# ebiggers/libdeflate

Measured on AMD Instinct MI355X. Metric: compress+decompress MB/s, 64 KiB chunks level 6, higher is better.
Workload: dtype u8

## Files before the change

### include/libdeflate_amd.h

```cpp
#ifndef LIBDEFLATE_AMD_H
#define LIBDEFLATE_AMD_H

#include <stddef.h>
#include <stdint.h>

#ifdef __cplusplus
extern "C" {
#endif

#define LIBDEFLATE_VERSION_MAJOR	1
#define LIBDEFLATE_VERSION_MINOR	25
#define LIBDEFLATE_VERSION_STRING	"1.25"
#define LIBDEFLATE_AMD_VERSION_STRING	"0.1-gfx950"

#ifndef LIBDEFLATEAPI
#  define LIBDEFLATEAPI __attribute__((visibility("default")))
#endif

struct libdeflate_compressor;
struct libdeflate_decompressor;

struct libdeflate_options {
	size_t sizeof_options;
	void *(*malloc_func)(size_t);
// ... 141 lines not shown
			      uint64_t *d_out_nbytes, void *stream);

LIBDEFLATEAPI int
libdeflate_amd_compress_batch_bounded(struct libdeflate_compressor *compressor,
				      int format, size_t n_chunks,
				      const void *d_in, const uint64_t *d_in_offsets,
				      const uint64_t *d_in_nbytes,
				      void *d_out, const uint64_t *d_out_offsets,
				      const uint64_t *d_out_avail,
				      uint64_t *d_out_nbytes, size_t max_in_nbytes,
				      void *stream);

LIBDEFLATEAPI void
libdeflate_amd_compress_last_schedule(const struct libdeflate_compressor *compressor,
				      uint32_t out[4]);

LIBDEFLATEAPI int
libdeflate_amd_decompress_batch(struct libdeflate_decompressor *decompressor,
				int format, size_t n_chunks,
				const void *d_in, const uint64_t *d_in_offsets,
				const uint64_t *d_in_nbytes,
				void *d_out, const uint64_t *d_out_offsets,
				const uint64_t *d_out_avail,
				int32_t *d_results,
				uint64_t *d_actual_in, uint64_t *d_actual_out,
				void *stream);

#define LIBDEFLATE_AMD_DICT_WINDOW 20480

LIBDEFLATEAPI int
// ... 439 lines not shown
```

### libdeflate_amd/api.py

```python
import collections
import ctypes
from ctypes import c_size_t, c_void_p

import numpy as np

from . import binding
from .binding import FORMATS, PREFIX, check


def _buf(b):
    if isinstance(b, np.ndarray):
        assert b.dtype == np.uint8 and b.flags["C_CONTIGUOUS"]
        return b.ctypes.data_as(c_void_p), b.size
    if isinstance(b, (bytes, bytearray, memoryview)):
        arr = np.frombuffer(b, dtype=np.uint8)
        return arr.ctypes.data_as(c_void_p), arr.size
    raise TypeError(type(b))


TarGz = collections.namedtuple("TarGz", "result nbytes seek_index windows words rows results")


class Compressor:

# ... 227 lines not shown
                self._h, FORMATS[fmt], in_offsets.numel(), data.data_ptr(),
                in_offsets.data_ptr(), in_nbytes.data_ptr(), out.data_ptr(),
                out_offsets.data_ptr(), out_avail.data_ptr(),
                out_nbytes.data_ptr(), _stream_ptr(stream)), "compress_batch")
        else:
            check(self._lib.libdeflate_amd_compress_batch_bounded(
                self._h, FORMATS[fmt], in_offsets.numel(), data.data_ptr(),
                in_offsets.data_ptr(), in_nbytes.data_ptr(), out.data_ptr(),
                out_offsets.data_ptr(), out_avail.data_ptr(),
                out_nbytes.data_ptr(), int(max_chunk), _stream_ptr(stream)),
                "compress_batch_bounded")

    def last_schedule(self):
        return binding.compress_last_schedule(self._h)

    def compress_dict(self, fmt, dictionary, data, out_avail=None):
        p, n = _buf(data)
        dp, dn = _buf(dictionary)
        if out_avail is None:
            out_avail = self.bound(fmt, n) + 4
        out = np.empty(max(out_avail, 1), dtype=np.uint8)
        r = self._lib.libdeflate_amd_compress_dict(
            self._h, FORMATS[fmt], dp, dn, p, n, out.ctypes.data_as(c_void_p), out_avail)
        if r == 0:
            return None
        return out[:r].tobytes()

    def compress_batch_dict(self, fmt, dictionary, data, in_offsets, in_nbytes, out,
                            out_offsets, out_avail, out_nbytes, stream=None):
        check(self._lib.libdeflate_amd_compress_batch_dict(
# ... 599 lines not shown
```

### libdeflate_amd/binding.py

```python
import ctypes
import os
from ctypes import (POINTER, c_char_p, c_int, c_int32, c_size_t, c_uint32,
                    c_uint64, c_void_p)

_HERE = os.path.dirname(os.path.abspath(__file__))
LIB_PATH = os.environ.get("LIBDEFLATE_AMD_LIB",
                          os.path.join(_HERE, "libdeflate_amd.so"))

SUCCESS, BAD_DATA, SHORT_OUTPUT, INSUFFICIENT_SPACE = 0, 1, 2, 3
FMT_DEFLATE, FMT_ZLIB, FMT_GZIP, FMT_BGZF = 0, 1, 2, 3
FORMATS = {"deflate": FMT_DEFLATE, "zlib": FMT_ZLIB, "gzip": FMT_GZIP, "bgzf": FMT_BGZF}
BGZF_BLOCK, BGZF_MEMBER_MAX, BGZF_EOF_BYTES, BGZF_NO_EOF = 65280, 65536, 28, 1
BGZF_MORE_MEMBERS, BGZF_HAS_EOF, BGZF_RESULT_WORDS, BGZF_VOFFSETS = 16, 1, 5, 2
GZM_MORE_MEMBERS, GZM_MORE_CANDIDATES, GZM_RESULT_WORDS, GZM_SLACK = 16, 17, 5, 1024
GZM_NAME_MAX = 65536
ZIP_MORE_ENTRIES, ZIP_MORE_CANDIDATES, ZIP_UNSUPPORTED = 16, 17, 18
ZIP_RESULT_WORDS, ZIP_WORDS, ZIP_SLACK, ZIP_ZIP64 = 5, 8, 1024, 1
ZIP_PIECE = 1 << 20
TAR_MORE_RECORDS, TAR_MORE_CANDIDATES, TAR_UNSUPPORTED = 16, 17, 18
TAR_RESULT_WORDS, TAR_WORDS, TAR_SLACK = 5, 8, 1024
TAR_EOF, TAR_HAS_L, TAR_HAS_PAX = 1, 2, 4
PNG_UNSUPPORTED, PNG_WORDS, PNG_LE16 = 18, 8, 1
PNG_FILTER_ADAPTIVE, PNGW_RESULT_WORDS = 5, 4
ZIP_STORE, ZIP_FORCE_ZIP64, ZIPW_RESULT_WORDS = 1, 2, 4
# ... 9 lines not shown
    "libdeflate_gzip_compress", "libdeflate_gzip_compress_bound",
    "libdeflate_free_compressor",
    "libdeflate_alloc_decompressor", "libdeflate_alloc_decompressor_ex",
    "libdeflate_deflate_decompress", "libdeflate_deflate_decompress_ex",
    "libdeflate_zlib_decompress", "libdeflate_zlib_decompress_ex",
    "libdeflate_gzip_decompress", "libdeflate_gzip_decompress_ex",
    "libdeflate_free_decompressor",
    "libdeflate_adler32", "libdeflate_crc32",
    "libdeflate_set_memory_allocator",
]
BATCH_SYMBOLS = [
    "libdeflate_amd_device_ready", "libdeflate_amd_last_error",
    "libdeflate_amd_reload_env",
    "libdeflate_amd_compress_batch", "libdeflate_amd_decompress_batch",
    "libdeflate_amd_compress_batch_bounded", "libdeflate_amd_compress_last_schedule",
    "libdeflate_amd_crc32_batch", "libdeflate_amd_adler32_batch",
    "libdeflate_amd_compress_batch_host",
    "libdeflate_amd_decompress_batch_host",
    "libdeflate_amd_compact_offsets_len", "libdeflate_amd_compact_batch",
    "libdeflate_amd_gzip_decompress_members",
    "libdeflate_amd_stream_stats", "libdeflate_amd_last_fanout",
    "libdeflate_amd_selfcheck",
    "libdeflate_amd_compress_batch_dict", "libdeflate_amd_decompress_batch_dict",
    "libdeflate_amd_compress_dict", "libdeflate_amd_decompress_dict_ex",
    "libdeflate_amd_bgzf_compress_bound", "libdeflate_amd_bgzf_compress_batch",
    "libdeflate_amd_bgzf_compress",
    "libdeflate_amd_bgzf_decompress_batch", "libdeflate_amd_bgzf_index_batch",
    "libdeflate_amd_bgzf_read_batch", "libdeflate_amd_bgzf_decompress",
    "libdeflate_amd_decompress_sizes_batch", "libdeflate_amd_decompress_sizes_batch_dict",
    "libdeflate_amd_decompress_sizes_batch_host", "libdeflate_amd_decompress_batch_packed",
# ... 58 lines not shown
        sig(f"libdeflate_{f}_decompress", c_int, P, P, SZ, P, SZ, psz)
        sig(f"libdeflate_{f}_decompress_ex", c_int, P, P, SZ, P, SZ, psz, psz)
    sig("libdeflate_crc32", c_uint32, c_uint32, P, SZ)
    sig("libdeflate_adler32", c_uint32, c_uint32, P, SZ)
    sig("libdeflate_set_memory_allocator", None, P, P)
    sig("libdeflate_amd_device_ready", c_int)
    sig("libdeflate_amd_last_error", c_char_p)
    sig("libdeflate_amd_reload_env", None)
    sig("libdeflate_amd_crc32_batch", c_int, SZ, P, P, P, P, P, P)
    sig("libdeflate_amd_adler32_batch", c_int, SZ, P, P, P, P, P, P)
    sig("libdeflate_amd_compress_batch", c_int, P, c_int, SZ, P, P, P, P, P,
        P, P, P)
    sig("libdeflate_amd_compress_batch_bounded", c_int, P, c_int, SZ, P, P, P, P, P,
        P, P, SZ, P)
    sig("libdeflate_amd_compress_last_schedule", None, P, POINTER(c_uint32))
    sig("libdeflate_amd_decompress_batch", c_int, P, c_int, SZ, P, P, P, P, P,
        P, P, P, P, P)
    sig("libdeflate_amd_compress_batch_host", c_int, P, c_int, SZ, P, P, P, P,
        P)
    sig("libdeflate_amd_decompress_batch_host", c_int, P, c_int, SZ, P, P, P,
        P, P, P, P)
    sig("libdeflate_amd_gzip_decompress_members", c_int, P, P, SZ, P, SZ, psz, psz, psz)
    sig("libdeflate_amd_stream_stats", None, POINTER(c_uint64))
    sig("libdeflate_amd_last_fanout", c_size_t)
    sig("libdeflate_amd_selfcheck", c_int, POINTER(c_uint64))
    sig("libdeflate_amd_compact_offsets_len", SZ, SZ)
    sig("libdeflate_amd_compact_batch", c_int, SZ, P, P, P, P, P, P)
    sig("libdeflate_amd_compress_batch_dict", c_int, P, c_int, SZ, P, SZ, P, P, P, P,
        P, P, P, P)
    sig("libdeflate_amd_decompress_batch_dict", c_int, P, c_int, SZ, P, SZ, P, P, P, P,
# ... 77 lines not shown
    out = (c_uint64 * 16)()
    load().libdeflate_amd_stream_stats(out)
    keys = ("parallel", "why_not", "filter_a", "blocks_found", "chunks_planned",
            "repairs", "chunks_decoded", "bytes", "us_in", "us_find", "us_count",
            "us_decode", "us_sum", "us_out", "windows", "host_chunks")
    return dict(zip(keys, [int(v) for v in out]))


def compress_last_schedule(compressor):
    out = (c_uint32 * 4)()
    load().libdeflate_amd_compress_last_schedule(compressor, out)
    return {"split": int(out[0]), "overlapped": int(out[1]), "head": int(out[2]),
            "tail": int(out[3])}


def last_error():
    return load().libdeflate_amd_last_error().decode()


def check(rc, what):
    if rc != 0:
        raise RuntimeError(f"{what} failed (status {rc}): {last_error()}")
```

### libdeflate_amd/csrc/deflate_kernel.hip

```cpp
#include <stddef.h>
#include "device_common.h"
#include "kernels.h"


#ifndef NT
#define NT LDA_DEFLATE_THREADS
#endif
#define VPT (1024 / NT)
#define NWAVES (NT / 64)
#ifndef TILE
#define TILE 4096
#endif
#ifndef RING
#define RING 32768u
#endif
#define RMASK (RING - 1)
#define LOOKAHEAD 272u
#ifndef HASH_BITS
#define HASH_BITS 13
#endif
#ifndef HASH3_BITS
#define HASH3_BITS 12
#endif
#define MAX_BLOCK_LEN 65536u
// ... 1414 lines not shown
	const u64 delta = ((u64)row16_sum(df >> 16) << 16) + row16_sum(df & 0xFFFF);
	bool sp = nprev && walkpos - block_start >= 5000 &&
		  delta >= (u64)nnew * 200 / 512 * nprev;
	if (fit_split && walkpos - block_start >= 5000)
		sp = true;
	wave_sync();
	if (lane < 10)
		L->obs[0][lane] = sp ? 0 : now;
	if (lane == 0)
		L->vars[V_SPLIT] = !sp ? 0 :
			L->vars[V_WPOS_PRE] - block_start >= 5000 ? 2 : 1;
}



static __device__ __forceinline__ u64 claim_buffer(lds_t *L, u32 *next_chunk, u32 tid)
{
	__syncthreads();
	if (tid == 0)
		L->vars[V_TMP0] = atomicAdd(next_chunk, 1u);
	__syncthreads();
	return bcast_first(L->vars[V_TMP0]);
}

static __device__ __forceinline__ void buffer_lds_init(lds_t *L, u32 tid)
{
	for (u32 i = tid; i < (1u << HASH_BITS) / 2; i += NT)
		((u32 *)L->head)[i] = 0x80008000u;
	for (u32 i = tid; i < (1u << HASH3_BITS) / 2; i += NT)
		((u32 *)L->head3)[i] = 0x80008000u;
	for (u32 i = tid; i < 320; i += NT)
		L->freq[i] = 0;
	if (tid < 10)
		L->obs[0][tid] = 0;
	if (tid < TILE / 64 + 1)
		L->rdy[tid] = 0;
	for (u32 i = tid; i < STG_WORDS + 8; i += NT)
		stg_of(L)[i] = 0;
	if (tid < 8)
		L->M[tid] = 0;
	if (tid == 0) {
		L->vars[V_NSEQ] = 0;
		L->vars[V_ENTRY] = 0;
		L->vars[V_PFLAG] = 0;
	}
// ... 103 lines not shown
{
	insert_tile3(L, c3ins, tnend,
		     tnend + TILE < n ? tnend + TILE : n, n, lane);
	__builtin_amdgcn_fence(__ATOMIC_RELEASE, "workgroup");
}

static __device__ __forceinline__ void
px_minlen_ahead(lds_t *L, u32 tnend, u32 n, u32 dict_len, u32 loaded, u32 depth, bool use3, u32 lane)
{
	const u32 nd = wave_distinct_bytes(L, tnend,
		loaded - tnend < TILE ? loaded - tnend : TILE, lane);
	if (lane == 0)
		L->vars[V_MINLEN] = min_len_policy(nd, n - dict_len, depth, use3);
}

static __device__ __forceinline__ void
px_round_b_tail(lds_t *L, u32 t, u32 n, u32 lo_nxt, u32 ml_cur, u32 depth, u32 nice,
		u32 mode, s32 limit, u32 tail_n, u32 tail_e, u32 tail_gen, u32 lane, u32 wave)
{
	__builtin_amdgcn_s_setprio(2);
	if (64 * (wave - 1) < tail_n) {
		u32 nx;
		(void)rb_batch(L, t, n, lo_nxt, ml_cur, rb_trim_depth(depth), nice,
			       tail_e, tail_e != 0, tail_gen, lane, &nx);
	}
	__builtin_amdgcn_fence(__ATOMIC_RELEASE, "workgroup");
	if (lane == 0)
		atomicAdd((u32 *)&L->vars[V_TAILDONE], 1u);
	wait_lds_eq(L, V_TAILDONE, RB_TAIL_WAVES);
	stage_steps_cur_claimed(L, limit, mode, nice, lane);
// ... 76 lines not shown
	const u8 *__restrict__ in_base, const u64 *__restrict__ in_offsets,    \
	const u64 *__restrict__ in_nbytes, u8 *__restrict__ out_base,          \
	const u64 *__restrict__ out_offsets,                                   \
	const u64 *__restrict__ out_avail_arr, u64 *__restrict__ out_nbytes,   \
	const u32 *__restrict__ sums, u64 *__restrict__ seq_scratch,           \
	const u32 *__restrict__ seg_info, u32 *__restrict__ next_chunk,       \
	const u8 *__restrict__ dict_pre
#define DEFLATE_KERNEL_ARGS                                                    \
	lds_raw, n_chunks, format, level, depth, nice, mode, in_base,          \
	in_offsets, in_nbytes, out_base, out_offsets, out_avail_arr,           \
	out_nbytes, sums, seq_scratch, seg_info, next_chunk, dict_pre

template <bool OPT, bool SPLIT = false> static __device__ __forceinline__ void
deflate_batch_body(u8 *lds_raw, DEFLATE_KERNEL_PARAMS,
		   u32 *__restrict__ tok_buf = NULL, u32 *__restrict__ blk_buf = NULL,
		   u32 tok_stride = 0, u32 blk_stride = 0, u32 *__restrict__ fused_cnt = NULL)
{
	static_assert(!(OPT && SPLIT), "levels 10-12 keep the fused block end");
	lds_t *L = (lds_t *)(uintptr_t)0;
	const u32 tid = threadIdx.x;
	if ((u32)(uintptr_t)(__attribute__((address_space(3))) u8 *)lds_raw != 0)
		__builtin_trap();
	u64 *__restrict__ seqg = seq_scratch + (size_t)blockIdx.x * SEQ_STRIDE;
	u32 *__restrict__ msave = (u32 *)(seqg + SEQ_GCAP);
	u32 *__restrict__ fsave = msave + TILE + 8;
	u32 *__restrict__ bsave = fsave + 640;
	u16 *__restrict__ c3g = (u16 *)(bsave + 512);
	u32 tog = 0;
	PROF_DECL;

	for (u32 i = tid; i < 256; i += NT) {
		u32 sl, xb, xv;
		length_code(i + 3, &sl, &xb, &xv);
		L->lslot[i] = (u8)sl;
	}
	const u32 *__restrict__ only = !SPLIT && blk_buf ? blk_buf + LDA_BLK_LIST(n_chunks) : NULL;
	const u64 n_todo = only ? bcast_first(*fused_cnt) : n_chunks;
	for (;;) {
		const u64 i_todo = claim_buffer(L, next_chunk, tid);
		if (i_todo >= n_todo)
			break;
		const u64 c = only ? bcast_first(only[i_todo]) : i_todo;
		const u8 *inp = in_base + in_offsets[c];
		u64 n64 = in_nbytes[c];
		u32 *__restrict__ const tokg = SPLIT ? tok_buf + c * tok_stride : (u32 *)seqg;
		u32 *__restrict__ const blk_desc = SPLIT ?
			blk_buf + LDA_BLK_HDR_WORDS(n_chunks) + c * blk_stride * LDA_BLK_WORDS : NULL;
		u32 nblocks = 0, blk_tok0 = 0;
		const u32 sinfo = dict_pre ? (n64 ? ((const u32 *)dict_pre)[0] : 0x80000000u) :
				  seg_info ? seg_info[c] : 0x80000000u;
		const u32 dict_len = sinfo & 0xFFFFu;
		const u32 lo_min = (sinfo >> 16) & 0x7FFFu;
		const bool seg_last = sinfo >> 31;
		const u32 pre_len = dict_pre ? dict_len : 0;
// ... 13 lines not shown
				overflow = true;
		}

		if (os.avail <= hdr_bytes + ftr_bytes && (hdr_bytes + ftr_bytes))
			overflow = true;
		if (n64 > 0xFFFFFF00u)
			overflow = true;
#ifdef LDA_SMALL
		if (n64 > RING)
			overflow = true;
#endif
		const bool over_bound = SPLIT && n64 > tok_stride;
		if (over_bound)
			overflow = true;
		const u32 n = (u32)n64;

		__syncthreads();
		PROF_START();
		buffer_lds_init(L, tid);
		os.sg = (u64)(0 - ((uintptr_t)os.out & 15));
		os.bits = 0;
		__syncthreads();

		if (!SPLIT) {
			if (!overflow && hdr_bytes)
				put_container_header(L, &os, format, level, dict_pre, hdr_bytes, tid);
			__syncthreads();
			stg_save(L, &os);
		}

		u32 loaded = 0;
		u32 block_start = dict_len;
		u32 walkpos = dict_len;
		const bool aligned_in = ((uintptr_t)inp & 15) == 0;

		const bool stored_only = level == 0 ||
			n - dict_len <= (u32)(55 - 4 * (level > 12 ? 12 : level));
		u32 num_tiles = (n + TILE - 1) / TILE;
		if (num_tiles == 0)
			num_tiles = 1;
		if (pre_len && !stored_only && !overflow) {
			stage_prefix(L, dict_pre + 64, pre_len, tid);
			loaded = pre_len;
		}

		const bool ra_all = depth <= 4;
		const bool optm = OPT && mode == 3;
		const u32 rounds = optm || ra_all ? 0 : S3_ROUNDS;
		const u32 dlim3 = mode ? 8192u : 4096u;
		const u32 ra_depth = ra_all ? depth : S3_RA_DEPTH;
		const u32 ra_class = ra_all ? DC_FULL :
				     ra_depth >= (depth >> S3_HALF_SHIFT) ? DC_HALF : DC_SHALLOW;
// ... 29 lines not shown
			} else {
				AS3 u32 *const MX = (AS3 u32 *)L->nxtB;
				const struct tile_window w = tile_window_of(t, tend, tn, lo_min, last_tile);
				u16 *c3nxt = c3g + (it & 1) * (TILE + 8);
				u16 *c3ins = c3g + ((it + 1) & 1) * (TILE + 8);

				const bool wl_copies = cur_real && !optm && rounds && mx_pending;
				if (cur_real) {
					cur_results_to_m(L, MX, fsave, mx_pending, wl_copies, carryv, walkpos, tid);
					mx_pending = false;
					ml_cur = ml_nxt;
					PROF_MARK(6);
				}
				const u32 s0_want0 = (it + 2) * TILE + LOOKAHEAD;
				const u32 s0_want = s0_want0 < n ? s0_want0 : n;
				const u32 s0_p = (loaded & ~15u) + tid * 16;
				const bool s0_pre = aligned_in && s0_p < s0_want;
				uint4 s0_v = make_uint4(0, 0, 0, 0);
				if (s0_pre)
					s0_v = *(const uint4 *)(inp + s0_p);
				tail_n = 0;
				if (cur_real && !optm) {
					if (rounds) {
						const u32 wc = build_worklist(L, (AS3 u32 *)L->nxtB,
									      wl_copies ? (const AS3 u32 *)MX : NULL,
									      mode, nice, wq_limit, tid);
						PROF_MARK(39);
						if (wc) {
							AS3 u32 *tl = (AS3 u32 *)L->nxtB;
							search_queue(L, t, n, w.lo_cur, ml_cur, depth, nice,
								     (AS3 u32 *)L->nxtB, (AS3 u32 *)L->nxtA, wc, tid,
								     nxt_real, &tail_n, &tail_gen, &tl);
							if (tail_n && wave >= 1 && wave <= RB_TAIL_WAVES) {
								const u32 k = 64 * (wave - 1) + lane;
								tail_e = k < tail_n ? tl[k] : 0;
// ... 65 lines not shown
							L->M[i] = msave[i];
						if (tid == 0) {
							L->vars[V_ENTRY] = ent0;
							L->vars[V_NSEQ] = nseq0;
						}
						__syncthreads();
						opt_stage++;
					}
				}

				const struct s0_state s0 = stage_s0(L, MX, inp, aligned_in, s0_pre, s0_p, s0_v,
					s0_want, loaded, ml_nxt, cur_real, nxt_real, tail_n, it, tid);
				loaded = s0.loaded;
				ml_nxt = s0.ml_nxt;
				PROF_MARK(1);
				if (it == 0) {
					if (wave == NWAVES - 1)
						insert_tile(L, 0, tnend, n, lane);
					if (wave == NWAVES - 2 && use3) {
						insert_tile3(L, c3nxt, 0, tnend, n, lane);
						__builtin_amdgcn_fence(__ATOMIC_RELEASE, "workgroup");
					}
					if (wave == NWAVES - 3 && nxt_real) {
						const u32 nd = wave_distinct_bytes(L, 0, loaded < TILE ? loaded : TILE, lane);
						if (lane == 0)
							L->vars[V_MINLEN] = min_len_policy(nd, n - dict_len, depth, use3);
					}
					__syncthreads();
					if (nxt_real)
						ml_nxt = bcast_first(L->vars[V_MINLEN]);
					PROF_MARK(2);
				}
				__builtin_amdgcn_fence(__ATOMIC_ACQUIRE, "workgroup");

				{
					const bool do_p2 = cur_real && !optm;
					AS3 u32 *const Mo = cur_real ? MX : (AS3 u32 *)L->M;
					PROF_WDECL;
					PROF_W0();
					if (wave == NWAVES - 1) {
						px_insert_chains(L, have_ins, tnend, n, lane);
						PROF_W(24);
					} else if (wave == NWAVES - 2) {
						__builtin_amdgcn_s_setprio(2);
						if (have_ins && use3)
							px_insert3(L, c3ins, tnend, n, lane);
						__builtin_amdgcn_s_setprio(0);
						if (have_ins && tnend >= dict_len)
							px_minlen_ahead(L, tnend, n, dict_len, loaded, depth, use3, lane);
						PROF_W(25);
					} else if (wave == 0 && do_p2) {
						if (tail_n)
							wait_lds_eq(L, V_ST2DONE, TILE / 64);
						__builtin_amdgcn_s_setprio(3);
						parse_and_base(L, tokg, t, w.limit, mode, nice, lane);
						__builtin_amdgcn_fence(__ATOMIC_RELEASE, "workgroup");
						if (lane == 0)
							*(volatile AS3 u32 *)&L->vars[V_PFLAG] = it;
						__builtin_amdgcn_s_setprio(0);
						if (tail_n && nxt_real && lane < 4)
							Mo[lane] = L->M[TILE + lane];
						PROF_W(26);
					} else if (RB_DEFER && tail_n && wave <= RB_TAIL_WAVES) {
						px_round_b_tail(L, t, n, w.lo_nxt, ml_cur, depth, nice, mode, w.limit,
// ... 148 lines not shown
			}
			carryv = 0;
			if (mx_pending) {
				mx_restore(L, msave, tid);
				mx_pending = false;
			}
			block_start = bend;
			__syncthreads();
		}

		if (SPLIT) {
			__syncthreads();
			if (tid == 0) {
				blk_buf[c] = over_bound ? LDA_BLK_FUSED :
					     overflow ? LDA_BLK_OVERFLOW : nblocks;
				if (over_bound)
					blk_buf[LDA_BLK_LIST(n_chunks) + atomicAdd(fused_cnt, 1u)] = (u32)c;
			}
		} else {
			finish_stream(L, &os, overflow, seg_last, format, ftr_bytes, sums, c, n,
				      out_nbytes, tid);
		}
	}
}

#ifdef LDA_SMALL
extern "C" __global__ void __launch_bounds__(NT, SMALL_WGS)
lda_deflate_small_kernel(DEFLATE_KERNEL_PARAMS)
{
	extern __shared__ __attribute__((aligned(16))) u8 lds_raw[];
// ... 8 lines not shown
extern "C" size_t lda_deflate_small_max(void)
{
	return RING;
}

extern "C" size_t lda_deflate_small_wgs(void)
{
	return SMALL_WGS;
}

LDA_PROF_DEFINE_READER(libdeflate_amd_profile_read_deflate_small)
#else
extern "C" __global__ void __launch_bounds__(NT)
lda_deflate_batch_kernel(DEFLATE_KERNEL_PARAMS, u32 *__restrict__ tok_buf,
			 u32 *__restrict__ blk_buf, u32 tok_stride, u32 blk_stride,
			 u32 *__restrict__ fused_cnt)
{
	extern __shared__ __attribute__((aligned(16))) u8 lds_raw[];
	deflate_batch_body<false, true>(DEFLATE_KERNEL_ARGS, tok_buf, blk_buf, tok_stride,
					blk_stride, fused_cnt);
}

extern "C" __global__ void __launch_bounds__(NT)
lda_deflate_fused_kernel(DEFLATE_KERNEL_PARAMS, const u32 *__restrict__ blk_buf,
			 const u32 *__restrict__ fused_cnt)
{
	extern __shared__ __attribute__((aligned(16))) u8 lds_raw[];
	deflate_batch_body<false>(DEFLATE_KERNEL_ARGS, NULL, (u32 *)blk_buf, 0, 0,
				  (u32 *)fused_cnt);
}

extern "C" __global__ void __launch_bounds__(NT)
lda_deflate_opt_kernel(DEFLATE_KERNEL_PARAMS)
{
	extern __shared__ __attribute__((aligned(16))) u8 lds_raw[];
// ... 22 lines not shown
```

### libdeflate_amd/csrc/host_common.h

```cpp
#ifndef LDA_HOST_COMMON_H
#define LDA_HOST_COMMON_H

#include <hip/hip_runtime.h>
#include <stddef.h>
#include <stdint.h>
#include <atomic>
#include <exception>
#include <functional>
#include <mutex>

#include "../../include/libdeflate_amd.h"

namespace lda {

void set_error(const char *fmt, ...);

#define LDA_HIP_TRY(expr, failret)                                           \
	do {                                                                 \
		hipError_t e_ = (expr);                                      \
		if (e_ != hipSuccess) {                                      \
			lda::set_error("%s: %s", #expr, hipGetErrorString(e_)); \
			return failret;                                      \
		}                                                            \
	} while (0)
// ... 38 lines not shown
	int inflate_waves_per_cu = 16;
	int sizes_waves_per_cu = 0;
	int host_threads = 4;
	size_t seg_bytes = 0;
	bool no_stream_par = false;
	size_t stream_par_min = 16384;
	size_t zip_large_min = (size_t)128 << 10;
	size_t stream_window = 0;
	size_t stream_chunk = 0;
	int devices = 1;
	bool no_selfcheck = false;
	bool bgzf_serial = false;
	bool tar_serial = false;
	bool fanout_oversub = false;
	bool compress_overlap = true;
	int compress_tail_rounds = 0;
};
const EnvCfg &env_cfg();

void *stage_reserve(DeviceCtx *ctx, size_t nbytes);

[[noreturn]] void die(const char *what);

void complain(const char *what, int status);

struct PinnedPair {
	uint8_t *buf[2] = { nullptr, nullptr };
	hipEvent_t ev[2] = { nullptr, nullptr };
	size_t cap = 0;
	bool ensure(size_t want);
// ... 95 lines not shown
```

### libdeflate_amd/csrc/host_compress.hip

```cpp
#include <stdio.h>
#include <stdlib.h>
#include <string.h>
#include <atomic>
#include <new>
#include <algorithm>
#include <vector>

#include "host_objects.h"
#include "kernels.h"
#include "large_plan.h"
#include "compress_plan.h"

using namespace lda;

struct level_cfg { uint32_t depth, nice, mode; };
static const level_cfg k_levels[13] = {
	{ 0, 0, 0 },
	{ 2, 32, 0 },
	{ 6, 10, 0 },
	{ 12, 14, 0 },
	{ 16, 30, 0 },
	{ 16, 30, 1 },
	{ 35, 65, 1 },
	{ 100, 130, 1 },
// ... 93 lines not shown
	return (32768 - 2 * tile - 272) / tile * tile;
}

struct dict_shape { uint32_t tail, pre_len, sinfo; };

static dict_shape shape_dict(int level, size_t dict_nbytes)
{
	const size_t tile = lda_deflate_tile();
	dict_shape d;
	d.tail = level == 0 ? 0 : (uint32_t)std::min(dict_nbytes, dict_window());
	d.pre_len = (uint32_t)((d.tail + tile - 1) / tile * tile);
	d.sinfo = d.pre_len | ((d.pre_len - d.tail) << 16) | 0x80000000u;
	return d;
}

static batch_plan plan_batch(const struct libdeflate_compressor *c, size_t n,
			     size_t max_in, bool seg, bool dict, bool overlap = true)
{
	static_assert(LDA_PLAN_BLK_WORDS == LDA_BLK_WORDS && LDA_PLAN_BLK_LIST(17) == LDA_BLK_LIST(17) &&
		      LDA_PLAN_BLK_HDR_WORDS(17) == LDA_BLK_HDR_WORDS(17), "compress_plan.h, kernels.h");
	const EnvCfg &env = env_cfg();
	compress_plan_env e;
	e.num_cus = (size_t)device_ctx()->num_cus;
	e.small_max = lda_deflate_small_max();
	e.small_wgs = lda_deflate_small_wgs();
	e.no_small = env.no_small;
	e.tile = lda_deflate_tile();
	e.seq_words = lda_deflate_seq_words();
	e.dict_bytes = LDA_DICT_BLK_HDR + dict_window();
	e.tail_rounds = !overlap || !env.compress_overlap || c->side.failed ? 0 :
// ... 28 lines not shown
	if (!c || !d_in || !d_in_offsets || !d_in_nbytes || !d_out ||
	    !d_out_offsets || !d_out_avail || !d_out_nbytes ||
	    format < LIBDEFLATE_AMD_DEFLATE || format > LIBDEFLATE_AMD_BGZF) {
		set_error("compress_batch: bad argument");
		return LIBDEFLATE_AMD_BAD_ARG;
	}
	const bool dict = d_dict && dict_nbytes;
	batch_plan pl = plan_batch(c, n, max_in_nbytes, d_seg_info != NULL, dict);
	if (pl.overlap && !c->side.ensure())
		pl = plan_batch(c, n, max_in_nbytes, d_seg_info != NULL, dict, false);
	const bool small = pl.small;
	c->last_schedule[0] = pl.split;
	c->last_schedule[1] = 0;
	c->last_schedule[2] = (uint32_t)std::min<size_t>(n, 0xFFFFFFFFu);
	c->last_schedule[3] = 0;
	uint8_t *scr = (uint8_t *)c->scratch.reserve(pl.total);
	if (!scr)
		return LIBDEFLATE_AMD_OOM;
	uint32_t *next_chunk = (uint32_t *)(scr + pl.cnt_at);
	LDA_HIP_TRY(hipMemsetAsync(next_chunk, 0, (pl.overlap ? 32 : 16) * pl.nslices, st),
		    LIBDEFLATE_AMD_NO_DEVICE);
	uint8_t *blk = NULL;
	if (dict) {
		const dict_shape sh = shape_dict(c->level, dict_nbytes);
		blk = scr + pl.dict_at;
		hipLaunchKernelGGL(lda_dict_prep_kernel, dim3(1), dim3(256), 0, st,
				   (const uint8_t *)d_dict, (uint64_t)dict_nbytes, sh.tail,
				   sh.pre_len, sh.sinfo, blk);
		LDA_HIP_TRY(hipGetLastError(), LIBDEFLATE_AMD_NO_DEVICE);
		if (format == LIBDEFLATE_AMD_ZLIB) {
// ... 64 lines not shown
		size_t lo, n;
		uint32_t *tok, *bd;
		uint32_t *cnt;
		uint64_t *seq;
		size_t grid_max;
	};
	auto lz77_entropy = [&](const part &q, hipStream_t on) -> int {
		const uint32_t *sk = sums ? sums + q.lo : NULL;
		const uint32_t *gk = d_seg_info ? d_seg_info + q.lo : NULL;
		hipLaunchKernelGGL(lda_deflate_batch_kernel, dim3((unsigned)std::min(q.n, q.grid_max)),
				   dim3(LDA_DEFLATE_THREADS), lds, on, (uint64_t)q.n, format,
				   c->level, lv.depth, lv.nice, lv.mode, (const uint8_t *)d_in,
				   d_in_offsets + q.lo, d_in_nbytes + q.lo, (uint8_t *)d_out,
				   d_out_offsets + q.lo, d_out_avail + q.lo, d_out_nbytes + q.lo, sk,
				   q.seq, gk, q.cnt, (const uint8_t *)NULL,
				   q.tok, q.bd, pl.tok_stride, pl.blk_stride, q.cnt + 2 * pl.nslices);
		LDA_HIP_TRY(hipGetLastError(), LIBDEFLATE_AMD_NO_DEVICE);
		hipLaunchKernelGGL(lda_deflate_entropy_kernel, dim3((unsigned)q.n),
				   dim3(LDA_DEFLATE_ENTROPY_THREADS), lda_deflate_entropy_lds_bytes(),
				   on, (uint64_t)q.n, format, c->level, (const uint8_t *)d_in,
				   d_in_offsets + q.lo, d_in_nbytes + q.lo, (uint8_t *)d_out,
				   d_out_offsets + q.lo, d_out_avail + q.lo, d_out_nbytes + q.lo, sk, gk,
				   (const uint32_t *)q.tok, (const uint32_t *)q.bd, pl.tok_stride,
				   pl.blk_stride, q.cnt + 3 * pl.nslices);
		LDA_HIP_TRY(hipGetLastError(), LIBDEFLATE_AMD_NO_DEVICE);
		return LIBDEFLATE_AMD_OK;
	};
	auto fused = [&](const part &q) -> int {
		const uint32_t *sk = sums ? sums + q.lo : NULL;
		const uint32_t *gk = d_seg_info ? d_seg_info + q.lo : NULL;
		hipLaunchKernelGGL(lda_deflate_fused_kernel, dim3((unsigned)std::min(q.n, pl.grid)),
// ... 8 lines not shown
		return LIBDEFLATE_AMD_OK;
	};
	size_t heads = 0, tails = 0;
	for (size_t k = 0; k < pl.nslices; k++) {
		const size_t lo = k * pl.per_slice, nk = std::min(pl.per_slice, n - lo);
		const size_t tail_n = plan_tail_of(nk, (size_t)ctx->num_cus, pl.tail_rounds);
		const size_t head_n = nk - tail_n;
		const part head = { lo, head_n, tok, (uint32_t *)(scr + pl.blk_at), next_chunk + k,
				    (uint64_t *)scr, pl.grid };
		const part tail = { lo + head_n, tail_n, tok + head_n * (size_t)pl.tok_stride,
				    (uint32_t *)(scr + pl.blk2_at),
				    (uint32_t *)(scr + pl.cnt2_at) + k,
				    (uint64_t *)(scr + pl.seq2_at), pl.grid2 };
		heads += head_n;
		tails += tail_n;
		if (tail_n) {
			LDA_HIP_TRY(hipEventRecord(c->side.in, st), LIBDEFLATE_AMD_NO_DEVICE);
			LDA_HIP_TRY(hipStreamWaitEvent(c->side.side, c->side.in, 0),
				    LIBDEFLATE_AMD_NO_DEVICE);
		}
		LDA_OK_TRY(lz77_entropy(head, st));
		if (tail_n) {
			const int rc = lz77_entropy(tail, c->side.side);
			LDA_HIP_TRY(hipEventRecord(c->side.tail, c->side.side), LIBDEFLATE_AMD_NO_DEVICE);
			LDA_HIP_TRY(hipStreamWaitEvent(st, c->side.tail, 0), LIBDEFLATE_AMD_NO_DEVICE);
			LDA_OK_TRY(rc);
		}
		LDA_OK_TRY(fused(head));
		if (tail_n)
			LDA_OK_TRY(fused(tail));
	}
	c->last_schedule[1] = tails != 0;
	c->last_schedule[2] = (uint32_t)std::min<size_t>(heads, 0xFFFFFFFFu);
	c->last_schedule[3] = (uint32_t)std::min<size_t>(tails, 0xFFFFFFFFu);
	return LIBDEFLATE_AMD_OK;
}

extern "C" LIBDEFLATEAPI void
libdeflate_amd_compress_last_schedule(const struct libdeflate_compressor *c, uint32_t out[4])
{
	for (int i = 0; i < 4; i++)
		out[i] = c ? c->last_schedule[i] : 0;
}

int lda::compress_deflate_pieces(struct libdeflate_compressor *c, size_t n, const void *d_in,
				 const uint64_t *d_in_offsets, const uint64_t *d_in_nbytes,
				 void *d_out, const uint64_t *d_out_offsets,
				 const uint64_t *d_out_avail, uint64_t *d_out_nbytes, void *stream,
				 const uint32_t *d_seg_info, size_t max_in)
{
	return compress_batch_impl(c, LIBDEFLATE_AMD_DEFLATE, n, d_in, d_in_offsets, d_in_nbytes,
				   d_out, d_out_offsets, d_out_avail, d_out_nbytes, stream,
				   d_seg_info, max_in);
}

size_t lda::compress_pieces_scratch(const struct libdeflate_compressor *c, size_t n,
				    size_t max_in, bool seg)
// ... 617 lines not shown
```

### libdeflate_amd/csrc/host_context.hip

```cpp
#include <stdarg.h>
#include <stdio.h>
#include <stdlib.h>
#include <string.h>
#include <pthread.h>
#include <algorithm>
#include <condition_variable>
#include <deque>
#include <functional>
#include <memory>
#include <thread>
#include <vector>

#include "host_common.h"
#include "kernels.h"

namespace lda {

static thread_local char g_err[512] = "";

void set_error(const char *fmt, ...)
{
	va_list ap;
	va_start(ap, fmt);
	vsnprintf(g_err, sizeof(g_err), fmt, ap);
// ... 64 lines not shown
	if (const char *e = getenv("LDA_DEVICES")) {
		if (!strcmp(e, "all")) {
			c.devices = -1;
		} else {
			int v = atoi(e);
			if (v >= 1 && v <= 16)
				c.devices = v;
		}
	}
	c.fanout_oversub = getenv("LDA_FANOUT_OVERSUB") != nullptr;
	c.no_selfcheck = getenv("LDA_NO_SELFCHECK") != nullptr;
	c.bgzf_serial = getenv("LDA_BGZF_SERIAL") != nullptr;
	c.tar_serial = getenv("LDA_TAR_SERIAL") != nullptr;
	if (const char *e = getenv("LDA_COMPRESS_OVERLAP"))
		c.compress_overlap = atoi(e) != 0;
	if (const char *e = getenv("LDA_COMPRESS_TAIL_ROUNDS")) {
		int v = atoi(e);
		if (v >= 1 && v <= 16)
			c.compress_tail_rounds = v;
	}
	return c;
}

static EnvCfg g_env = read_env();

const EnvCfg &env_cfg()
{
	return g_env;
}

// ... 726 lines not shown
```

### libdeflate_amd/csrc/host_objects.h

```cpp
#ifndef LDA_HOST_OBJECTS_H
#define LDA_HOST_OBJECTS_H

#include "host_common.h"
#include "stream_types.h"
#include <functional>

namespace lda {

typedef void *(*malloc_func_t)(size_t);
typedef void (*free_func_t)(void *);

extern malloc_func_t g_malloc;
extern free_func_t g_free;

struct DevBuf {
	void *p = nullptr;
	size_t cap = 0;
	void *reserve(size_t n);
	void release();
};

}

#define LDA_MAX_SHARDS 16
// ... 22 lines not shown
	lda::malloc_func_t malloc_func;
	int device;
	struct libdeflate_compressor *shard[LDA_MAX_SHARDS];
	int level;
	lda::DevBuf scratch;
	lda::DevBuf stage;
	lda::DevBuf bgzf;
	lda::DevBuf large;
	lda::DevBuf zipw;
	lda::Upload zipw_up;
	lda::PinnedPair pinned;
	lda::PinnedBuf meta;
	lda::StreamPair streams;
	lda::SideStream side;
	uint32_t last_schedule[4] = { 0, 0, 0, 0 };
};

namespace lda {
bool pick_allocator(const struct libdeflate_options *options,
		    malloc_func_t *m, free_func_t *f);

template <typename Obj>
int fanout(Obj *o, size_t n, const size_t *weight,
	   const std::function<Obj *(const struct libdeflate_options *)> &alloc,
	   const std::function<int(Obj *, size_t, size_t)> &body);

int compress_deflate_pieces(struct libdeflate_compressor *c, size_t n, const void *d_in,
			    const uint64_t *d_in_offsets, const uint64_t *d_in_nbytes, void *d_out,
			    const uint64_t *d_out_offsets, const uint64_t *d_out_avail,
			    uint64_t *d_out_nbytes, void *stream, const uint32_t *d_seg_info,
// ... 44 lines not shown
```

### libdeflate_amd/csrc/kernels.h

```cpp
#ifndef LDA_KERNELS_H
#define LDA_KERNELS_H

#include <hip/hip_runtime.h>
#include <stdint.h>

#include "large_plan.h"

extern "C" __global__ void
lda_crc32_batch_kernel(uint64_t n_chunks, const uint8_t *base,
		       const uint64_t *offsets, const uint64_t *nbytes,
		       const uint32_t *init, uint32_t *out,
		       const uint32_t *g_tables, const uint32_t *xpow8);
extern "C" __global__ void
lda_adler32_batch_kernel(uint64_t n_chunks, const uint8_t *base,
			 const uint64_t *offsets, const uint64_t *nbytes,
			 const uint32_t *init, uint32_t *out);
#define LDA_DICT_BLK_HDR 64
extern "C" __global__ void
lda_dict_prep_kernel(const uint8_t *dict, uint64_t dict_nbytes, uint32_t tail,
		     uint32_t pre_len, uint32_t sinfo, uint8_t *blk);

extern "C" __global__ void
lda_inflate_batch_kernel(uint64_t n_chunks, int format, uint32_t lpw,
			 const uint8_t *in_base,
// ... 47 lines not shown
extern "C" size_t lda_inflate_tokcap(void);
extern "C" size_t lda_inflate_window_bytes(void);
extern "C" __global__ void
lda_inflate_finalize_kernel(uint64_t n_chunks, int format, int exact_fill,
			    const uint8_t *in_base, const uint64_t *in_offsets,
			    const uint64_t *out_avail, const uint32_t *sums,
			    int32_t *results, uint64_t *actual_in,
			    uint64_t *actual_out);

#define LDA_DEFLATE_THREADS 1024
#define LDA_BLK_TOK0 0
#define LDA_BLK_NTOK 1
#define LDA_BLK_START 2
#define LDA_BLK_END 3
#define LDA_BLK_FLAGS 4
#define LDA_BLK_STORED 2u
#define LDA_BLK_FREQ 8
#define LDA_BLK_WORDS (LDA_BLK_FREQ + 320)
#define LDA_BLK_OVERFLOW 0xFFFFFFFFu
#define LDA_BLK_FUSED 0xFFFFFFFEu
#define LDA_BLK_LIST(n) (((n) + 15) / 16 * 16)
#define LDA_BLK_HDR_WORDS(n) (2 * LDA_BLK_LIST(n))
extern "C" __global__ void
lda_deflate_batch_kernel(uint64_t n_chunks, int format, int level,
			 uint32_t depth, uint32_t nice, uint32_t mode,
			 const uint8_t *in_base, const uint64_t *in_offsets,
			 const uint64_t *in_nbytes, uint8_t *out_base,
			 const uint64_t *out_offsets, const uint64_t *out_avail,
			 uint64_t *out_nbytes, const uint32_t *sums,
			 uint64_t *seq_scratch, const uint32_t *seg_info,
			 uint32_t *next_chunk, const uint8_t *dict_pre,
			 uint32_t *tok_buf, uint32_t *blk_buf, uint32_t tok_stride,
			 uint32_t blk_stride, uint32_t *fused_cnt);
extern "C" __global__ void
lda_deflate_fused_kernel(uint64_t n_chunks, int format, int level,
			 uint32_t depth, uint32_t nice, uint32_t mode,
			 const uint8_t *in_base, const uint64_t *in_offsets,
			 const uint64_t *in_nbytes, uint8_t *out_base,
			 const uint64_t *out_offsets, const uint64_t *out_avail,
			 uint64_t *out_nbytes, const uint32_t *sums,
			 uint64_t *seq_scratch, const uint32_t *seg_info,
			 uint32_t *next_chunk, const uint8_t *dict_pre,
			 const uint32_t *blk_buf, const uint32_t *fused_cnt);
#define LDA_DEFLATE_ENTROPY_THREADS 256
extern "C" __global__ void
lda_deflate_entropy_kernel(uint64_t n_chunks, int format, int level,
			   const uint8_t *in_base, const uint64_t *in_offsets,
			   const uint64_t *in_nbytes, uint8_t *out_base,
// ... 377 lines not shown
```

Measured before the change: 34940.

## Carry LZ77 prep across chunks: prefetch and hash-insert next chunk's first tile

In the split deflate kernel, a workgroup claims its next chunk ahead of time during the second-to-last tile. During the last tile it prefetches that chunk's first tile, clears the hash tables and inserts the new chunk's first tile. The next iteration then skips the table reset and the initial tile load and insert, which removes per-chunk startup cost and serialisation between chunks. This adds complexity and extra branches in the last tiles, and it applies only when the tile count is a multiple of the ring size and level is 8 or below. A debug query for the number of carried chunks is also added.

```diff
diff --git a/include/libdeflate_amd.h b/include/libdeflate_amd.h
--- a/include/libdeflate_amd.h
+++ b/include/libdeflate_amd.h
@@ -179,6 +179,10 @@
 LIBDEFLATEAPI void
 libdeflate_amd_compress_last_schedule(const struct libdeflate_compressor *compressor,
 				      uint32_t out[4]);
+
+LIBDEFLATEAPI int
+libdeflate_amd_compress_last_carry(const struct libdeflate_compressor *compressor,
+				   uint32_t *out);
 
 LIBDEFLATEAPI int
 libdeflate_amd_decompress_batch(struct libdeflate_decompressor *decompressor,
diff --git a/libdeflate_amd/api.py b/libdeflate_amd/api.py
--- a/libdeflate_amd/api.py
+++ b/libdeflate_amd/api.py
@@ -265,6 +265,9 @@
     def last_schedule(self):
         return binding.compress_last_schedule(self._h)
 
+    def last_carry(self):
+        return binding.compress_last_carry(self._h)
+
     def compress_dict(self, fmt, dictionary, data, out_avail=None):
         p, n = _buf(data)
         dp, dn = _buf(dictionary)
diff --git a/libdeflate_amd/binding.py b/libdeflate_amd/binding.py
--- a/libdeflate_amd/binding.py
+++ b/libdeflate_amd/binding.py
@@ -47,6 +47,7 @@
     "libdeflate_amd_reload_env",
     "libdeflate_amd_compress_batch", "libdeflate_amd_decompress_batch",
     "libdeflate_amd_compress_batch_bounded", "libdeflate_amd_compress_last_schedule",
+    "libdeflate_amd_compress_last_carry",
     "libdeflate_amd_crc32_batch", "libdeflate_amd_adler32_batch",
     "libdeflate_amd_compress_batch_host",
     "libdeflate_amd_decompress_batch_host",
@@ -135,6 +136,7 @@
     sig("libdeflate_amd_compress_batch_bounded", c_int, P, c_int, SZ, P, P, P, P, P,
         P, P, SZ, P)
     sig("libdeflate_amd_compress_last_schedule", None, P, POINTER(c_uint32))
+    sig("libdeflate_amd_compress_last_carry", c_int, P, POINTER(c_uint32))
     sig("libdeflate_amd_decompress_batch", c_int, P, c_int, SZ, P, P, P, P, P,
         P, P, P, P, P)
     sig("libdeflate_amd_compress_batch_host", c_int, P, c_int, SZ, P, P, P, P,
@@ -242,6 +244,12 @@
             "tail": int(out[3])}
 
 
+def compress_last_carry(compressor):
+    out = (c_uint32 * 1)()
+    check(load().libdeflate_amd_compress_last_carry(compressor, out), "compress_last_carry")
+    return int(out[0])
+
+
 def last_error():
     return load().libdeflate_amd_last_error().decode()
 
diff --git a/libdeflate_amd/csrc/deflate_kernel.hip b/libdeflate_amd/csrc/deflate_kernel.hip
--- a/libdeflate_amd/csrc/deflate_kernel.hip
+++ b/libdeflate_amd/csrc/deflate_kernel.hip
@@ -1452,6 +1452,11 @@
 
 
 
+static __device__ __forceinline__ bool stored_only_of(int level, u32 nbytes)
+{
+	return level == 0 || nbytes <= (u32)(55 - 4 * (level > 12 ? 12 : level));
+}
+
 static __device__ __forceinline__ u64 claim_buffer(lds_t *L, u32 *next_chunk, u32 tid)
 {
 	__syncthreads();
@@ -1461,12 +1466,14 @@
 	return bcast_first(L->vars[V_TMP0]);
 }
 
-static __device__ __forceinline__ void buffer_lds_init(lds_t *L, u32 tid)
-{
-	for (u32 i = tid; i < (1u << HASH_BITS) / 2; i += NT)
-		((u32 *)L->head)[i] = 0x80008000u;
-	for (u32 i = tid; i < (1u << HASH3_BITS) / 2; i += NT)
-		((u32 *)L->head3)[i] = 0x80008000u;
+static __device__ __forceinline__ void buffer_lds_init(lds_t *L, u32 tid, bool keep_tables = false)
+{
+	if (!keep_tables) {
+		for (u32 i = tid; i < (1u << HASH_BITS) / 2; i += NT)
+			((u32 *)L->head)[i] = 0x80008000u;
+		for (u32 i = tid; i < (1u << HASH3_BITS) / 2; i += NT)
+			((u32 *)L->head3)[i] = 0x80008000u;
+	}
 	for (u32 i = tid; i < 320; i += NT)
 		L->freq[i] = 0;
 	if (tid < 10)
@@ -1600,6 +1607,52 @@
 		L->vars[V_MINLEN] = min_len_policy(nd, n - dict_len, depth, use3);
 }
 
+
+enum { NX_IDX = 0, NX_OFF_LO, NX_OFF_HI, NX_NBYTES, NX_STATE, NX_PREP };
+
+static __device__ __forceinline__ void
+px_claim_ahead(lds_t *L, u32 *next_chunk, u64 n_todo, const u64 *__restrict__ in_offsets,
+	       const u64 *__restrict__ in_nbytes, u32 lane)
+{
+	if (lane == 0) {
+		const u32 i = atomicAdd(next_chunk, 1u);
+		u64 off = 0, nb = 0;
+		if (i < n_todo) {
+			off = in_offsets[i];
+			nb = in_nbytes[i];
+		}
+		L->carry[NX_IDX] = i;
+		L->carry[NX_OFF_LO] = (u32)off;
+		L->carry[NX_OFF_HI] = (u32)(off >> 32);
+		L->carry[NX_NBYTES] = nb > 0xFFFFFFFFu ? 0xFFFFFFFFu : (u32)nb;
+	}
+}
+
+struct seam_next {
+	bool ok;
+	const u8 *src;
+	u32 n;
+};
+
+static __device__ __forceinline__ struct seam_next
+seam_next_of(lds_t *L, u64 n_todo, const u8 *__restrict__ in_base)
+{
+	struct seam_next r = { false, in_base, 0 };
+	if (bcast_first(L->carry[NX_STATE])) {
+		r.src = in_base + mk64(bcast_first(L->carry[NX_OFF_LO]),
+				       bcast_first(L->carry[NX_OFF_HI]));
+		r.n = bcast_first(L->carry[NX_NBYTES]);
+		r.ok = bcast_first(L->carry[NX_IDX]) < n_todo && ((uintptr_t)r.src & 15) == 0;
+	}
+	return r;
+}
+
+static __device__ __forceinline__ void px_clear_table(AS3 u32 *tab, u32 words, u32 lane)
+{
+	for (u32 i = lane; i < words; i += 64)
+		tab[i] = 0x80008000u;
+}
+
 static __device__ __forceinline__ void
 px_round_b_tail(lds_t *L, u32 t, u32 n, u32 lo_nxt, u32 ml_cur, u32 depth, u32 nice,
 		u32 mode, s32 limit, u32 tail_n, u32 tail_e, u32 tail_gen, u32 lane, u32 wave)
@@ -1706,7 +1759,8 @@
 template <bool OPT, bool SPLIT = false> static __device__ __forceinline__ void
 deflate_batch_body(u8 *lds_raw, DEFLATE_KERNEL_PARAMS,
 		   u32 *__restrict__ tok_buf = NULL, u32 *__restrict__ blk_buf = NULL,
-		   u32 tok_stride = 0, u32 blk_stride = 0, u32 *__restrict__ fused_cnt = NULL)
+		   u32 tok_stride = 0, u32 blk_stride = 0, u32 *__restrict__ fused_cnt = NULL,
+		   u32 lz77_carry = 0)
 {
 	static_assert(!(OPT && SPLIT), "levels 10-12 keep the fused block end");
 	lds_t *L = (lds_t *)(uintptr_t)0;
@@ -1728,8 +1782,15 @@
 	}
 	const u32 *__restrict__ only = !SPLIT && blk_buf ? blk_buf + LDA_BLK_LIST(n_chunks) : NULL;
 	const u64 n_todo = only ? bcast_first(*fused_cnt) : n_chunks;
+	if (SPLIT) {
+		if (tid == 0)
+			L->carry[NX_STATE] = 0;
+		__syncthreads();
+	}
 	for (;;) {
-		const u64 i_todo = claim_buffer(L, next_chunk, tid);
+		const u32 nxs = SPLIT ? bcast_first(L->carry[NX_STATE]) : 0;
+		const u64 i_todo = SPLIT && nxs ? (u64)bcast_first(L->carry[NX_IDX]) :
+				   claim_buffer(L, next_chunk, tid);
 		if (i_todo >= n_todo)
 			break;
 		const u64 c = only ? bcast_first(only[i_todo]) : i_todo;
@@ -1773,10 +1834,19 @@
 		if (over_bound)
 			overflow = true;
 		const u32 n = (u32)n64;
+		const bool prepared = SPLIT && nxs == 2 && !overflow &&
+				      !stored_only_of(level, n - dict_len);
 
 		__syncthreads();
 		PROF_START();
-		buffer_lds_init(L, tid);
+		buffer_lds_init(L, tid, prepared);
+		if (SPLIT && tid == 0) {
+			const u32 nt = (n + TILE - 1) / TILE;
+			L->carry[NX_STATE] = lz77_carry && !dict_pre && !seg_info && !overflow &&
+					     !stored_only_of(level, n - dict_len) &&
+					     nt >= RING / TILE && nt % (RING / TILE) == 0;
+			L->carry[NX_PREP] = prepared;
+		}
 		os.sg = (u64)(0 - ((uintptr_t)os.out & 15));
 		os.bits = 0;
 		__syncthreads();
@@ -1788,13 +1858,12 @@
 			stg_save(L, &os);
 		}
 
-		u32 loaded = 0;
+		u32 loaded = !prepared ? 0 : n < TILE + LOOKAHEAD ? n : TILE + LOOKAHEAD;
 		u32 block_start = dict_len;
 		u32 walkpos = dict_len;
 		const bool aligned_in = ((uintptr_t)inp & 15) == 0;
 
-		const bool stored_only = level == 0 ||
-			n - dict_len <= (u32)(55 - 4 * (level > 12 ? 12 : level));
+		const bool stored_only = stored_only_of(level, n - dict_len);
 		u32 num_tiles = (n + TILE - 1) / TILE;
 		if (num_tiles == 0)
 			num_tiles = 1;
@@ -1854,11 +1923,20 @@
 				}
 				const u32 s0_want0 = (it + 2) * TILE + LOOKAHEAD;
 				const u32 s0_want = s0_want0 < n ? s0_want0 : n;
-				const u32 s0_p = (loaded & ~15u) + tid * 16;
-				const bool s0_pre = aligned_in && s0_p < s0_want;
+				u32 s0_p = (loaded & ~15u) + tid * 16;
+				bool s0_pre = aligned_in && s0_p < s0_want;
 				uint4 s0_v = make_uint4(0, 0, 0, 0);
 				if (s0_pre)
 					s0_v = *(const uint4 *)(inp + s0_p);
+				if (SPLIT && it + 1 == num_tiles) {
+					const struct seam_next nx = seam_next_of(L, n_todo, in_base);
+					if (nx.ok) {
+						s0_p = tid * 16;
+						s0_pre = s0_p < (nx.n < TILE + LOOKAHEAD ? nx.n : TILE + LOOKAHEAD);
+						if (s0_pre)
+							s0_v = *(const uint4 *)(nx.src + s0_p);
+					}
+				}
 				tail_n = 0;
 				if (cur_real && !optm) {
 					if (rounds) {
@@ -1954,7 +2032,9 @@
 				loaded = s0.loaded;
 				ml_nxt = s0.ml_nxt;
 				PROF_MARK(1);
-				if (it == 0) {
+				if (SPLIT && it == 0 && bcast_first(L->carry[NX_PREP])) {
+					ml_nxt = bcast_first(L->vars[V_MINLEN]);
+				} else if (it == 0) {
 					if (wave == NWAVES - 1)
 						insert_tile(L, 0, tnend, n, lane);
 					if (wave == NWAVES - 2 && use3) {
@@ -1979,15 +2059,42 @@
 					PROF_WDECL;
 					PROF_W0();
 					if (wave == NWAVES - 1) {
-						px_insert_chains(L, have_ins, tnend, n, lane);
+						bool ins = have_ins;
+						u32 ins_t = tnend, ins_n = n;
+						if (SPLIT && it + 1 == num_tiles) {
+							const struct seam_next nx = seam_next_of(L, n_todo, in_base);
+							if (nx.ok) {
+								px_clear_table((AS3 u32 *)L->head, (1u << HASH_BITS) / 2, lane);
+								ins = true;
+								ins_t = 0;
+								ins_n = nx.n;
+							}
+						}
+						px_insert_chains(L, ins, ins_t, ins_n, lane);
 						PROF_W(24);
 					} else if (wave == NWAVES - 2) {
+						bool ins = have_ins;
+						u32 ins_t = tnend, ins_n = n, ins_loaded = loaded;
+						if (SPLIT && it + 1 == num_tiles) {
+							const struct seam_next nx = seam_next_of(L, n_todo, in_base);
+							if (nx.ok) {
+								px_clear_table((AS3 u32 *)L->head3, (1u << HASH3_BITS) / 2, lane);
+								if (lane == 0)
+									L->carry[NX_STATE] = 2;
+								ins = true;
+								ins_t = 0;
+								ins_n = nx.n;
+								ins_loaded = nx.n < TILE + LOOKAHEAD ? nx.n : TILE + LOOKAHEAD;
+							}
+						}
 						__builtin_amdgcn_s_setprio(2);
-						if (have_ins && use3)
-							px_insert3(L, c3ins, tnend, n, lane);
+						if (ins && use3)
+							px_insert3(L, c3ins, ins_t, ins_n, lane);
 						__builtin_amdgcn_s_setprio(0);
-						if (have_ins && tnend >= dict_len)
-							px_minlen_ahead(L, tnend, n, dict_len, loaded, depth, use3, lane);
+						if (ins && ins_t >= dict_len)
+							px_minlen_ahead(L, ins_t, ins_n, dict_len, ins_loaded, depth, use3, lane);
+						if (SPLIT && it + 2 == num_tiles && bcast_first(L->carry[NX_STATE]))
+							px_claim_ahead(L, next_chunk, n_todo, in_offsets, in_nbytes, lane);
 						PROF_W(25);
 					} else if (wave == 0 && do_p2) {
 						if (tail_n)
@@ -2166,6 +2273,7 @@
 			if (tid == 0) {
 				blk_buf[c] = over_bound ? LDA_BLK_FUSED :
 					     overflow ? LDA_BLK_OVERFLOW : nblocks;
+				blk_desc[LDA_BLK_CARRIED] = L->carry[NX_PREP];
 				if (over_bound)
 					blk_buf[LDA_BLK_LIST(n_chunks) + atomicAdd(fused_cnt, 1u)] = (u32)c;
 			}
@@ -2204,11 +2312,11 @@
 extern "C" __global__ void __launch_bounds__(NT)
 lda_deflate_batch_kernel(DEFLATE_KERNEL_PARAMS, u32 *__restrict__ tok_buf,
 			 u32 *__restrict__ blk_buf, u32 tok_stride, u32 blk_stride,
-			 u32 *__restrict__ fused_cnt)
+			 u32 *__restrict__ fused_cnt, u32 lz77_carry)
 {
 	extern __shared__ __attribute__((aligned(16))) u8 lds_raw[];
 	deflate_batch_body<false, true>(DEFLATE_KERNEL_ARGS, tok_buf, blk_buf, tok_stride,
-					blk_stride, fused_cnt);
+					blk_stride, fused_cnt, lz77_carry);
 }
 
 extern "C" __global__ void __launch_bounds__(NT)
diff --git a/libdeflate_amd/csrc/host_common.h b/libdeflate_amd/csrc/host_common.h
--- a/libdeflate_amd/csrc/host_common.h
+++ b/libdeflate_amd/csrc/host_common.h
@@ -76,6 +76,7 @@
 	bool tar_serial = false;
 	bool fanout_oversub = false;
 	bool compress_overlap = true;
+	bool lz77_carry = true;
 	int compress_tail_rounds = 0;
 };
 const EnvCfg &env_cfg();
diff --git a/libdeflate_amd/csrc/host_compress.hip b/libdeflate_amd/csrc/host_compress.hip
--- a/libdeflate_amd/csrc/host_compress.hip
+++ b/libdeflate_amd/csrc/host_compress.hip
@@ -131,6 +131,8 @@
 	return d;
 }
 
+#define LDA_LZ77_CARRY_MAX_LEVEL 8
+
 static batch_plan plan_batch(const struct libdeflate_compressor *c, size_t n,
 			     size_t max_in, bool seg, bool dict, bool overlap = true)
 {
@@ -189,6 +191,7 @@
 	c->last_schedule[1] = 0;
 	c->last_schedule[2] = (uint32_t)std::min<size_t>(n, 0xFFFFFFFFu);
 	c->last_schedule[3] = 0;
+	c->last_parts[0] = c->last_parts[1] = { NULL, 0, 0 };
 	uint8_t *scr = (uint8_t *)c->scratch.reserve(pl.total);
 	if (!scr)
 		return LIBDEFLATE_AMD_OOM;
@@ -283,7 +286,8 @@
 				   d_in_offsets + q.lo, d_in_nbytes + q.lo, (uint8_t *)d_out,
 				   d_out_offsets + q.lo, d_out_avail + q.lo, d_out_nbytes + q.lo, sk,
 				   q.seq, gk, q.cnt, (const uint8_t *)NULL,
-				   q.tok, q.bd, pl.tok_stride, pl.blk_stride, q.cnt + 2 * pl.nslices);
+				   q.tok, q.bd, pl.tok_stride, pl.blk_stride, q.cnt + 2 * pl.nslices,
+				   (uint32_t)(env_cfg().lz77_carry && c->level <= LDA_LZ77_CARRY_MAX_LEVEL));
 		LDA_HIP_TRY(hipGetLastError(), LIBDEFLATE_AMD_NO_DEVICE);
 		hipLaunchKernelGGL(lda_deflate_entropy_kernel, dim3((unsigned)q.n),
 				   dim3(LDA_DEFLATE_ENTROPY_THREADS), lda_deflate_entropy_lds_bytes(),
@@ -322,6 +326,9 @@
 				    (uint64_t *)(scr + pl.seq2_at), pl.grid2 };
 		heads += head_n;
 		tails += tail_n;
+		const size_t pitch = (size_t)pl.blk_stride * LDA_BLK_WORDS;
+		c->last_parts[0] = { head.bd + LDA_BLK_HDR_WORDS(head_n), head_n, pitch };
+		c->last_parts[1] = { tail.bd + LDA_BLK_HDR_WORDS(tail_n), tail_n, pitch };
 		if (tail_n) {
 			LDA_HIP_TRY(hipEventRecord(c->side.in, st), LIBDEFLATE_AMD_NO_DEVICE);
 			LDA_HIP_TRY(hipStreamWaitEvent(c->side.side, c->side.in, 0),
@@ -349,6 +356,31 @@
 {
 	for (int i = 0; i < 4; i++)
 		out[i] = c ? c->last_schedule[i] : 0;
+}
+
+extern "C" LIBDEFLATEAPI int
+libdeflate_amd_compress_last_carry(const struct libdeflate_compressor *c, uint32_t *out)
+{
+	if (!c || !out) {
+		set_error("compress_last_carry: bad argument");
+		return LIBDEFLATE_AMD_BAD_ARG;
+	}
+	DeviceGuard on(c->device);
+	if (!on.ok())
+		return LIBDEFLATE_AMD_NO_DEVICE;
+	LDA_HIP_TRY(hipDeviceSynchronize(), LIBDEFLATE_AMD_NO_DEVICE);
+	uint32_t sum = 0;
+	for (const auto &q : c->last_parts) {
+		if (!q.n)
+			continue;
+		std::vector<uint32_t> col(q.n);
+		LDA_HIP_TRY(hipMemcpy2D(col.data(), 4, q.desc + LDA_BLK_CARRIED, q.pitch * 4, 4, q.n,
+					hipMemcpyDeviceToHost), LIBDEFLATE_AMD_NO_DEVICE);
+		for (uint32_t v : col)
+			sum += v != 0;
+	}
+	*out = sum;
+	return LIBDEFLATE_AMD_OK;
 }
 
 int lda::compress_deflate_pieces(struct libdeflate_compressor *c, size_t n, const void *d_in,
diff --git a/libdeflate_amd/csrc/host_context.hip b/libdeflate_amd/csrc/host_context.hip
--- a/libdeflate_amd/csrc/host_context.hip
+++ b/libdeflate_amd/csrc/host_context.hip
@@ -102,6 +102,8 @@
 	c.tar_serial = getenv("LDA_TAR_SERIAL") != nullptr;
 	if (const char *e = getenv("LDA_COMPRESS_OVERLAP"))
 		c.compress_overlap = atoi(e) != 0;
+	if (const char *e = getenv("LDA_LZ77_CARRY"))
+		c.lz77_carry = atoi(e) != 0;
 	if (const char *e = getenv("LDA_COMPRESS_TAIL_ROUNDS")) {
 		int v = atoi(e);
 		if (v >= 1 && v <= 16)
diff --git a/libdeflate_amd/csrc/host_objects.h b/libdeflate_amd/csrc/host_objects.h
--- a/libdeflate_amd/csrc/host_objects.h
+++ b/libdeflate_amd/csrc/host_objects.h
@@ -60,6 +60,7 @@
 	lda::StreamPair streams;
 	lda::SideStream side;
 	uint32_t last_schedule[4] = { 0, 0, 0, 0 };
+	struct { const uint32_t *desc; size_t n, pitch; } last_parts[2] = {};
 };
 
 namespace lda {
diff --git a/libdeflate_amd/csrc/kernels.h b/libdeflate_amd/csrc/kernels.h
--- a/libdeflate_amd/csrc/kernels.h
+++ b/libdeflate_amd/csrc/kernels.h
@@ -85,6 +85,7 @@
 #define LDA_BLK_START 2
 #define LDA_BLK_END 3
 #define LDA_BLK_FLAGS 4
+#define LDA_BLK_CARRIED 5
 #define LDA_BLK_STORED 2u
 #define LDA_BLK_FREQ 8
 #define LDA_BLK_WORDS (LDA_BLK_FREQ + 320)
@@ -102,7 +103,7 @@
 			 uint64_t *seq_scratch, const uint32_t *seg_info,
 			 uint32_t *next_chunk, const uint8_t *dict_pre,
 			 uint32_t *tok_buf, uint32_t *blk_buf, uint32_t tok_stride,
-			 uint32_t blk_stride, uint32_t *fused_cnt);
+			 uint32_t blk_stride, uint32_t *fused_cnt, uint32_t lz77_carry);
 extern "C" __global__ void
 lda_deflate_fused_kernel(uint64_t n_chunks, int format, int level,
 			 uint32_t depth, uint32_t nice, uint32_t mode,
```

Result: no change. 35170, median of 6 (+0.7%).
